# chaoyang223/UDA

Measured on AMD Instinct MI355X. Metric: TeraSort shuffle+merge GB/s whole-node, higher is better.
Workload: dtype bytes

## Files before the change

csrc/gpu/colpack.hip:

```cpp
#include "codec/colpack.h"
#include "kernels.h"

#include <algorithm>

namespace uda {
namespace gpu {

namespace {
constexpr int kCpThreads = 256;
constexpr int kCpTileRows = 128;
constexpr int kCpTileBytes = kCpTileRows * (9 * kColpackMaxRecordBytes / 10);
constexpr int kCpTableDelta = 2 * kColpackMaxRecordBytes;
constexpr int kCpTableStride = kCpTableDelta + 2 * kColpackMaxKeyBytes;

__device__ __forceinline__ uint64_t load_cols(const uint8_t* p, int n) {
  if (n == 8 && (reinterpret_cast<uintptr_t>(p) & 7) == 0) return *reinterpret_cast<const uint64_t*>(p);
  uint64_t x = 0;
  for (int k = 0; k < n; ++k) x |= (uint64_t)p[k] << (8 * k);
  return x;
}

struct Key128 {
  uint64_t hi, lo;
};
// ... 29 lines not shown
#pragma unroll
  for (int c = 0; c < 8; ++c) {
    const int col = 8 * g + c;
    if (col >= ko && col < ko + kl) {
      const int j = ko + kl - 1 - col;
      const uint64_t b = (j < 8 ? t.lo >> (8 * j) : t.hi >> (8 * (j - 8))) & 0xFF;
      x = (x & ~(0xFFull << (8 * c))) | (b << (8 * c));
    }
  }
  return x;
}

__device__ __forceinline__ bool group_has_key(int g, int ko, int kl) { return kl > 0 && 8 * g < ko + kl && 8 * g + 8 > ko; }

__global__ void __launch_bounds__(kCpThreads) colpack_stats_kernel(const ColpackPieceDesc* pieces, int L,
                                                                   uint32_t buf_records, int ko, int kl,
                                                                   uint32_t* table) {
  const ColpackPieceDesc pc = pieces[blockIdx.y];
  const int G = (L + 7) / 8;
  const int rows_per_iter = kCpThreads / G;
  if ((int64_t)blockIdx.x * rows_per_iter >= pc.nrec) return;
  __shared__ uint32_t s_mn[kColpackMaxRecordBytes], s_mx[kColpackMaxRecordBytes];
  __shared__ uint32_t s_dmn[kColpackMaxKeyBytes], s_dmx[kColpackMaxKeyBytes];
  const int t = threadIdx.x;
  s_mn[t] = 255;
  s_mx[t] = 0;
  if (t < kColpackMaxKeyBytes) {
    s_dmn[t] = 255;
    s_dmx[t] = 0;
  }
  __syncthreads();
  const int g = t % G, rl = t / G;
  if (rl < rows_per_iter) {
    const int ncol = min(8, L - 8 * g);
    const bool keyed = group_has_key(g, ko, kl);
    uint32_t mn[8], mx[8], dmn[8], dmx[8];
#pragma unroll
    for (int c = 0; c < 8; ++c) {
      mn[c] = dmn[c] = 255;
      mx[c] = dmx[c] = 0;
    }
    const uint8_t* p = pc.src + 8 * g;
    const int64_t step = (int64_t)gridDim.x * rows_per_iter;
#pragma unroll 4
    for (int64_t r = (int64_t)blockIdx.x * rows_per_iter + rl; r < pc.nrec; r += step) {
      const uint64_t x = load_cols(p + r * L, ncol);
#pragma unroll
      for (int c = 0; c < 8; ++c) {
        const uint32_t v = (uint32_t)(x >> (8 * c)) & 0xFF;
        mn[c] = min(mn[c], v);
        mx[c] = max(mx[c], v);
      }
      if (keyed) {
        const uint64_t xd = with_key_delta(x, g, key_delta(pc.src + r * L, r, L, buf_records, ko, kl), ko, kl);
#pragma unroll
        for (int c = 0; c < 8; ++c) {
          const uint32_t v = (uint32_t)(xd >> (8 * c)) & 0xFF;
          dmn[c] = min(dmn[c], v);
          dmx[c] = max(dmx[c], v);
        }
      }
    }
#pragma unroll
    for (int c = 0; c < 8; ++c)
      if (c < ncol) {
        atomicMin(&s_mn[8 * g + c], mn[c]);
        atomicMax(&s_mx[8 * g + c], mx[c]);
        const int kc = 8 * g + c - ko;
        if (keyed && kc >= 0 && kc < kl) {
          atomicMin(&s_dmn[kc], dmn[c]);
          atomicMax(&s_dmx[kc], dmx[c]);
        }
      }
  }
  __syncthreads();
  uint32_t* tb = table + (size_t)blockIdx.y * kCpTableStride;
  if (t < L) {
    atomicMin(&tb[t], s_mn[t]);
    atomicMin(&tb[kColpackMaxRecordBytes + t], 255u - s_mx[t]);
  }
  if (t < kl) {
    atomicMin(&tb[kCpTableDelta + t], s_dmn[t]);
    atomicMin(&tb[kCpTableDelta + kColpackMaxKeyBytes + t], 255u - s_dmx[t]);
  }
}

__device__ __forceinline__ int width_of(uint32_t mn, uint32_t mx) {
  const uint32_t range = mx > mn ? mx - mn : 0;
  return range ? 32 - __clz((int)range) : 0;
}

__global__ void __launch_bounds__(64) colpack_plan_kernel(const ColpackPieceDesc* pieces, int L, uint32_t buf_records,
                                                          uint32_t version, int ko, int kl, const uint32_t* table,
                                                          ColpackResult* results) {
  const ColpackPieceDesc pc = pieces[blockIdx.x];
  const uint32_t* tb = table + (size_t)blockIdx.x * kCpTableStride;
// ... 158 lines not shown

void launch_colpack(const ColpackPieceDesc* pieces, int npieces, int64_t max_nrec, int L, int64_t buf_records,
                    uint32_t* table, ColpackResult* results, hipStream_t s, int version, int key_off, int key_len) {
  if (npieces <= 0) return;
  if (version != (int)kColpackVersion2) version = (int)kColpackVersion, key_len = 0;
  if (key_len <= 0 || key_len > kColpackMaxKeyBytes || key_off < 0 || key_off + key_len > L || buf_records < 1 ||
      buf_records > 0xFFFFFFFFll)
    key_len = 0;
  if (key_len == 0) key_off = 0;
  (void)hipMemsetAsync(table, 0xFF, colpack_table_bytes(npieces), s);
  const int G = (L + 7) / 8;
  const int rows_per_iter = kCpThreads / G;
  int64_t sb = (max_nrec + (int64_t)rows_per_iter * 32 - 1) / ((int64_t)rows_per_iter * 32);
  sb = std::max<int64_t>(1, std::min<int64_t>(sb, 256));
  hipLaunchKernelGGL(colpack_stats_kernel, dim3((unsigned)sb, (unsigned)npieces), dim3(kCpThreads), 0, s, pieces, L,
                     (uint32_t)buf_records, key_off, key_len, table);
  hipLaunchKernelGGL(colpack_plan_kernel, dim3((unsigned)npieces), dim3(64), 0, s, pieces, L, (uint32_t)buf_records,
                     (uint32_t)version, key_off, key_len, table, results);
  int64_t pb = (max_nrec + kCpTileRows - 1) / kCpTileRows;
  pb = std::max<int64_t>(1, std::min<int64_t>(pb, 1024));
  if (G == 13)
    hipLaunchKernelGGL(colpack_pack_kernel<13>, dim3((unsigned)pb, (unsigned)npieces), dim3(kCpThreads), 0, s, pieces, L);
  else
    hipLaunchKernelGGL(colpack_pack_kernel<0>, dim3((unsigned)pb, (unsigned)npieces), dim3(kCpThreads), 0, s, pieces, L);
}

}
}
```

csrc/gpu/delivery_schedule.cc:

```cpp
#include "delivery_schedule.h"

#include <algorithm>
#include <stdexcept>

namespace uda {
namespace gpu {

void check_delivery_order(const std::string& order) {
  if (order != "wave" && order != "reducer") throw std::runtime_error("delivery_order must be wave or reducer");
}

std::vector<DeliveryPiece> delivery_schedule(const std::vector<int64_t>& group_recs, int64_t piece_bytes,
                                             const std::string& order, int64_t record_bytes) {
  check_delivery_order(order);
  if (record_bytes < 1) throw std::runtime_error("delivery_schedule: record_bytes < 1");
  const int64_t piece = std::max<int64_t>(1, piece_bytes / record_bytes) * record_bytes;
  std::vector<DeliveryPiece> v;
  std::vector<size_t> first(group_recs.size() + 1, 0);
  int64_t goff = 0;
  size_t waves = 0;
  for (size_t i = 0; i < group_recs.size(); ++i) {
    if (group_recs[i] < 0) throw std::runtime_error("delivery_schedule: negative record count");
    const int64_t bytes = group_recs[i] * record_bytes;
    for (int64_t off = 0; off < bytes;) {
      const int64_t len = std::min(piece, bytes - off);
      off += len;
      v.push_back(DeliveryPiece{(int)i, goff + off - len, len, (int)v.size(), off >= bytes});
    }
    goff += bytes;
    first[i + 1] = v.size();
    waves = std::max(waves, first[i + 1] - first[i]);
  }
  if (order == "reducer") return v;
  std::vector<DeliveryPiece> w;
  w.reserve(v.size());
  for (size_t k = 0; k < waves; ++k)
    for (size_t i = 0; i < group_recs.size(); ++i)
      if (first[i] + k < first[i + 1]) w.push_back(v[first[i] + k]);
  return w;
}

}
}
```

csrc/gpu/delivery_schedule.h:

```cpp
#pragma once
#include <cstdint>
#include <string>
#include <vector>

namespace uda {
namespace gpu {

struct DeliveryPiece {
  int reducer;
  int64_t src_off;
  int64_t len;
  int pack_index;
  bool last_of_reducer;
};

void check_delivery_order(const std::string& order);

std::vector<DeliveryPiece> delivery_schedule(const std::vector<int64_t>& group_recs, int64_t piece_bytes,
                                             const std::string& order, int64_t record_bytes = 104);

}
}
```

csrc/gpu/device_engine.cc:

```cpp
#include "device_engine.h"
#include "codec/colpack.h"
#include "device_ptr.h"
#include "hbm_ledger.h"
#include "merge_plan.h"
#include "sdma.h"
#include "uda/fault.h"
#include "uda/topology.h"
#include "uda/trace.h"

#include <rccl/rccl.h>
#include <unistd.h>

#include <algorithm>
#include <atomic>
#include <chrono>
#include <cstring>
#include <map>
#include <mutex>
#include <numeric>
#include <stdexcept>

#include "uda/log.h"
#include "uda/vint.h"
#include "uda/thread_name.h"
// ... 694 lines not shown
}

ShuffleJob::ShuffleJob(const ShuffleConfig& cfg) : cfg_(cfg) {
  if (cfg_.world < 1 || cfg_.rank < 0 || cfg_.rank >= cfg_.world)
    throw std::runtime_error("ShuffleJob: bad rank/world");
  if (cfg_.maps_per_rank < 1) throw std::runtime_error("ShuffleJob: maps_per_rank < 1");
  if (cfg_.rounds < 1) cfg_.rounds = 1;
  if (cfg_.reducers < 1) cfg_.reducers = 1;
  if (cfg_.pinned_slots < 2) cfg_.pinned_slots = 2;
  if (cfg_.d2h != "sdma" && cfg_.d2h != "hip") throw std::runtime_error("ShuffleJob: d2h must be sdma or hip");
  if (cfg_.store != "hbm" && cfg_.store != "host" && cfg_.store != "disk")
    throw std::runtime_error("unknown store tier " + cfg_.store);
  if (cfg_.delivery_pack != "auto" && cfg_.delivery_pack != "v1" && cfg_.delivery_pack != "off")
    throw std::runtime_error("ShuffleJob: delivery_pack must be auto, v1 or off");
  check_delivery_order(cfg_.delivery_order);
  pack_ = cfg_.deliver_host && cfg_.delivery_pack != "off";
  pack_version_ = cfg_.delivery_pack == "v1" ? (int)kColpackVersion : (int)kColpackVersion2;
  if (const char* e = std::getenv("UDA_DELIVERY_PACK"))
    if (std::atoi(e) == 0) pack_ = false;
  R_ = cfg_.reducers;
  Q_ = cfg_.rounds;
  C_ = R_ * Q_;
  if ((int64_t)R_ * cfg_.world * cfg_.maps_per_rank > 65536)
    throw std::runtime_error("ShuffleJob: reducers * world * maps_per_rank must be <= 65536 (merge run index)");
  HIP_CHECK(hipSetDevice(cfg_.device));
  int lo_prio = 0, hi_prio = 0;
  HIP_CHECK(hipDeviceGetStreamPriorityRange(&lo_prio, &hi_prio));
  const bool spill = cfg_.store != "hbm";
  HIP_CHECK(hipStreamCreateWithPriority(&s_comm_, hipStreamNonBlocking, spill ? lo_prio : hi_prio));
  HIP_CHECK(hipStreamCreateWithPriority(&s_compute_, hipStreamNonBlocking, spill ? hi_prio : lo_prio));
  HIP_CHECK(hipStreamCreateWithFlags(&s_copy_, hipStreamNonBlocking));
  HIP_CHECK(hipStreamCreateWithFlags(&s_plan_, hipStreamNonBlocking));
  buf_records_ = std::max<int64_t>(1, cfg_.kv_buf_bytes / kTeraRecordBytes);
  const int64_t buf_bytes = buf_records_ * kTeraRecordBytes;
  piece_bytes_ = std::max<int64_t>(1, cfg_.d2h_piece_bytes / buf_bytes) * buf_bytes;
  ring_stride_ = pack_ ? std::max(piece_bytes_, pack_bound(piece_bytes_ / kTeraRecordBytes)) : piece_bytes_;
  merged_ev_.resize(kSlots);
  comm_ev_.resize(kSlots);
  sent_ev_.resize(2);
  early_ev_.resize(kSlots);
  for (auto& e : early_ev_) HIP_CHECK(hipEventCreateWithFlags(&e, hipEventDisableTiming));
  for (auto& e : merged_ev_) HIP_CHECK(hipEventCreateWithFlags(&e, hipEventDisableTiming));
  for (auto& e : comm_ev_) HIP_CHECK(hipEventCreateWithFlags(&e, hipEventDisableTiming));
  for (auto& e : sent_ev_) HIP_CHECK(hipEventCreateWithFlags(&e, hipEventDisableTiming));
}

ShuffleJob::~ShuffleJob() {
  {
    std::lock_guard<std::mutex> g(mu_);
    stop_ = true;
  }
  cv_.notify_all();
  if (copy_thr_.joinable()) copy_thr_.join();
  for (auto& t : consumers_)
    if (t.joinable()) t.join();
  (void)hipDeviceSynchronize();
  for (auto e : merged_ev_) (void)hipEventDestroy(e);
  for (auto e : early_ev_) (void)hipEventDestroy(e);
  if (s_stage_) (void)hipStreamDestroy(s_stage_);
  for (auto e : comm_ev_) (void)hipEventDestroy(e);
  for (auto e : sent_ev_) (void)hipEventDestroy(e);
  for (auto e : piece_ev_) (void)hipEventDestroy(e);
  if (!sdma_ && ring_) pinned_host_free(ring_);
  if (sdma_) {
    for (auto sg : piece_sig_) sdma_->destroy_signal(sg);
    sdma_->free_host(ring_);
    ring_ = nullptr;
    sdma_.reset();
  }
  exchange_.reset();
  if (s_copy_) (void)hipStreamDestroy(s_copy_);
  if (s_plan_) (void)hipStreamDestroy(s_plan_);
  if (s_comm_) (void)hipStreamDestroy(s_comm_);
// ... 10 lines not shown
  if (cfg_.world == 1) return;
  if (cfg_.local_group.empty()) throw std::runtime_error("init_local: config.local_group is empty");
  HIP_CHECK(hipSetDevice(cfg_.device));
  exchange_ = make_local_exchange(cfg_.local_group, cfg_.rank, cfg_.world);
}

void ShuffleJob::init_ipc(const std::string& name) {
  if (cfg_.world == 1) return;
  HIP_CHECK(hipSetDevice(cfg_.device));
  exchange_ = make_ipc_exchange(name, cfg_.rank, cfg_.world, cfg_.device);
}

std::string ShuffleJob::delivery_name() const {
  if (!cfg_.deliver_host) return "none";
  std::string name = sdma_ ? sdma_->describe() : "hip[numa=" + std::to_string(device_numa_node(cfg_.device)) + "]";
  name += " ring=" + ring_numa_ + " order=" + cfg_.delivery_order;
  if (!pack_) return name + " pack=off";
  name += " pack=colbits v" + std::to_string(pack_version_);
  if (last_delta_ >= 0) name += last_delta_ ? " delta" : " plain";
  if (last_d2h_ratio_ >= 0) {
    char b[32];
    std::snprintf(b, sizeof(b), " d2h/in=%.3f", last_d2h_ratio_);
    name += b;
  }
  return name;
}

int64_t ShuffleJob::pack_bound(int64_t nrec) const {
  return pack_version_ == (int)kColpackVersion ? colpack_bound(kTeraRecordBytes, nrec)
                                               : colpack2_bound(kTeraRecordBytes, nrec, buf_records_);
}

std::vector<ShuffleJob::PackPiece> ShuffleJob::round_pieces(const std::vector<int64_t>& group_recs) const {
  std::vector<PackPiece> v;
  int64_t doff = 0;
  for (const DeliveryPiece& dp : delivery_schedule(group_recs, piece_bytes_, "reducer", kTeraRecordBytes)) {
    const int64_t nrec = dp.len / kTeraRecordBytes;
    v.push_back(PackPiece{dp.src_off, doff, nrec});
    doff += pack_bound(nrec);
  }
  return v;
}

void ShuffleJob::note_issue(int k, double now) {
  if (first_issue_ms_ < 0) first_issue_ms_ = now;
  if (flying_ == 0 && idle_since_ms_ >= 0) step_link_idle_ms_ += now - idle_since_ms_;
  slot_flying_[k] = true;
  ++flying_;
}

void ShuffleJob::note_landing(int k, double now) {
// ... 416 lines not shown
      }
      verify_n_[q] = (int)vruns[q].size();
    }
  }

  merger_.reset(new DeviceMerger(max_round_records_, R_ * W * M));
  const size_t out_bytes = (size_t)std::max<int64_t>(1, max_round_records_) * kTeraRecordBytes;
  out_slots_.clear();
  out_slots_.resize(kSlots);
  for (auto& b : out_slots_) b.alloc(out_bytes);
  packed_slots_.clear();
  d_pack_pieces_.clear();
  d_pack_results_.clear();
  h_pack_results_.clear();
  pack_n_.assign(Q_, 0);
  pack_max_nrec_.assign(Q_, 0);
  pack_early_.assign(Q_, 0);
  if (pack_) {
    int64_t packed_bytes = 64;
    int max_pieces = 1;
    std::vector<std::vector<PackPiece>> pieces(Q_);
    for (int q = 0; q < Q_; ++q) {
      pieces[q] = round_pieces(plans_[q].group_recs);
      if (pieces[q].size() > 65535) throw std::runtime_error("delivery_pack: more than 65535 D2H pieces in a round");
      pack_n_[q] = (int)pieces[q].size();
      max_pieces = std::max(max_pieces, pack_n_[q]);
      for (const PackPiece& pc : pieces[q]) {
        pack_max_nrec_[q] = std::max(pack_max_nrec_[q], pc.nrec);
        packed_bytes = std::max(packed_bytes, pc.dst_off + pack_bound(pc.nrec));
      }
    }
    packed_slots_.resize(kSlots);
    for (auto& b : packed_slots_) b.alloc((size_t)packed_bytes);
    d_pack_results_.resize(kSlots);
    h_pack_results_.resize(kSlots);
    for (int k = 0; k < kSlots; ++k) {
      d_pack_results_[k].alloc((size_t)max_pieces * sizeof(ColpackResult));
      h_pack_results_[k].alloc((size_t)max_pieces * sizeof(ColpackResult));
    }
    d_pack_table_.alloc(colpack_table_bytes(max_pieces));
    d_pack_pieces_.resize(Q_);
    for (int q = 0; q < Q_; ++q) {
      if (pieces[q].empty()) continue;
      std::vector<ColpackPieceDesc> v;
      int wave0 = 0;
      for (const DeliveryPiece& dp :
           delivery_schedule(plans_[q].group_recs, piece_bytes_, cfg_.delivery_order, kTeraRecordBytes)) {
        const PackPiece& pc = pieces[q][(size_t)dp.pack_index];
        v.push_back(ColpackPieceDesc{out_slots_[q % kSlots].as<uint8_t>() + pc.src_off,
                                     packed_slots_[q % kSlots].as<uint8_t>() + pc.dst_off, pc.nrec});
      }
      for (int64_t g : plans_[q].group_recs) wave0 += g > 0 ? 1 : 0;
      if (cfg_.delivery_order == "wave" && wave0 < pack_n_[q]) pack_early_[q] = wave0;
      d_pack_pieces_[q].alloc(v.size() * sizeof(ColpackPieceDesc));
      HIP_CHECK(hipMemcpy(d_pack_pieces_[q].as(), v.data(), v.size() * sizeof(ColpackPieceDesc), hipMemcpyHostToDevice));
    }
  }
  recv_slots_.clear();
  if (staged()) {
    recv_slots_.resize(kSlots);
    for (auto& b : recv_slots_) b.alloc((size_t)std::max<int64_t>(max_slot_bytes, 16));
  }
  for (auto& b : send_staging_) b.reset();
  if (W > 1 && spilled())
    for (auto& b : send_staging_) b.alloc((size_t)std::max<int64_t>(max_send, 16));
  if (W > 1) exchange_->reserve(max_send);
  for (int q = 0; q < Q_; ++q) {
    RoundPlan& rp = plans_[q];
// ... 156 lines not shown
}

void ShuffleJob::copy_loop() {
  try {
    bind_thread_to_cpus(device_consumer_cpus(cfg_.device));
    HIP_CHECK(hipSetDevice(cfg_.device));
    for (;;) {
      RoundOut r;
      {
        std::unique_lock<std::mutex> lk(mu_);
        cv_.wait(lk, [&] { return stop_ || !round_q_.empty(); });
        if (stop_) return;
        r = std::move(round_q_.front());
        round_q_.pop_front();
      }
      HIP_CHECK(hipEventSynchronize(r.early > 0 ? early_ev_[r.slot] : merged_ev_[r.slot]));
      const uint8_t* src = out_slots_[r.slot].as<uint8_t>();
      const bool last_round = (r.q == Q_ - 1);
      bool check;
      {
        std::lock_guard<std::mutex> g(mu_);
        check = step_check_delivery_;
      }
      if (check) {
        std::vector<RunDesc> gr(R_);
        int64_t o = 0, mx = 0;
        for (int i = 0; i < R_; ++i) {
          gr[i].base = src + o * kTeraRecordBytes;
          gr[i].nrec = r.group_recs[i];
          gr[i].nbytes = gr[i].nrec * kTeraRecordBytes;
          gr[i].offsets = nullptr;
          o += r.group_recs[i];
          mx = std::max(mx, r.group_recs[i]);
        }
        std::vector<uint64_t> ck(R_, 0);
        HIP_CHECK(hipMemcpyAsync(d_d2h_runs_.as(), gr.data(), (size_t)R_ * sizeof(RunDesc), hipMemcpyHostToDevice, s_copy_));
        launch_slice_checksums(d_d2h_runs_.as<RunDesc>(), R_, std::max<int64_t>(mx, 1),
                               d_d2h_ck_.as<unsigned long long>(), s_copy_);
        HIP_CHECK(hipGetLastError());
        HIP_CHECK(hipMemcpyAsync(ck.data(), d_d2h_ck_.as(), (size_t)R_ * 8, hipMemcpyDeviceToHost, s_copy_));
        HIP_CHECK(hipStreamSynchronize(s_copy_));
        std::lock_guard<std::mutex> g(mu_);
        for (int i = 0; i < R_; ++i) pre_d2h_ck_[(size_t)r.q * R_ + i] = ck[i];
      }
      std::vector<int> used;
      const std::vector<PackPiece> ppieces = pack_ ? round_pieces(r.group_recs) : std::vector<PackPiece>();
      const ColpackResult* pres = pack_ ? h_pack_results_[r.slot].as<ColpackResult>() : nullptr;
      if (last_round) {
        bool any = false;
        {
          std::lock_guard<std::mutex> g(mu_);
          for (int i = 0; i < R_; ++i)
            if (r.group_recs[i] == 0) {
              items_[i].push_back(Item{-1, 0, true, now_ms(), r.q});
              any = true;
            }
        }
        if (any) cv_.notify_all();
      }
      int issued = 0;
      for (const DeliveryPiece& dp :
           delivery_schedule(r.group_recs, piece_bytes_, cfg_.delivery_order, kTeraRecordBytes)) {
        if (r.early > 0 && issued == r.early) HIP_CHECK(hipEventSynchronize(merged_ev_[r.slot]));
        int k = -1;
        {
          std::unique_lock<std::mutex> lk(mu_);
          auto have_slot = [&] {
            if (stop_) return true;
            for (bool f : pinned_free_)
              if (f) return true;
            return false;
          };
          if (!have_slot()) {
            const double tw = now_ms();
            while (!cv_.wait_for(lk, std::chrono::microseconds(200), have_slot)) poll_landings();
            step_slot_wait_ms_ += now_ms() - tw;
          }
          if (stop_) return;
// ... 546 lines not shown
      int64_t goff = 0;
      for (int i = 0; i < R_; ++i) {
        const int64_t g = rp.group_recs[i];
        if (g > 0) {
          launch_validate_fixed(out + goff * kTeraRecordBytes, g, vprev + i, has_prev[i] ? 1 : 0, vlast + i, vstats,
                                s_compute_, dg + 4 + i);
          HIP_CHECK(hipMemcpyAsync(vprev + i, vlast + i, sizeof(Elem), hipMemcpyDeviceToDevice, s_compute_));
          has_prev[i] = true;
        }
        goff += g;
      }
      check_inputs(1);
    }
    HIP_CHECK(hipEventRecord(ev[4 * q + 3], s_compute_));
    if (pack_ && deliver && pack_n_[q] > 0) {
      auto pack_range = [&](int a, int b) {
        launch_colpack(d_pack_pieces_[q].as<ColpackPieceDesc>() + a, b - a, pack_max_nrec_[q], kTeraRecordBytes,
                       buf_records_, d_pack_table_.as<uint32_t>(), d_pack_results_[slot].as<ColpackResult>() + a,
                       s_compute_, pack_version_, kTeraKeyOffset, kTeraKeyBytes);
        HIP_CHECK(hipGetLastError());
        HIP_CHECK(hipMemcpyAsync(h_pack_results_[slot].as<ColpackResult>() + a,
                                 d_pack_results_[slot].as<ColpackResult>() + a, (size_t)(b - a) * sizeof(ColpackResult),
                                 hipMemcpyDeviceToHost, s_compute_));
      };
      if (pack_early_[q] > 0) {
        pack_range(0, pack_early_[q]);
        HIP_CHECK(hipEventRecord(early_ev_[slot], s_compute_));
      }
      pack_range(pack_early_[q], pack_n_[q]);
    }
    HIP_CHECK(hipEventRecord(merged_ev_[slot], s_compute_));
    if (sdma_stage) {
      std::lock_guard<std::mutex> g(mu_);
      merge_recorded[q] = 1;
      cv_.notify_all();
    }
    st.records += n;
    if (deliver) {
      {
        std::lock_guard<std::mutex> g(mu_);
        round_q_.push_back(RoundOut{q, slot, rp.group_recs, pack_early_[q]});
      }
      cv_.notify_all();
    }
  }
  if (deliver) wait_until([&] { return eof_count_ == R_; });
  if (exchange_) exchange_->wait(s_comm_);
  HIP_CHECK(hipStreamSynchronize(s_compute_));
  HIP_CHECK(hipStreamSynchronize(s_comm_));
  HIP_CHECK(hipStreamSynchronize(s_copy_));
  if (stage_thr.joinable()) stage_thr.join();
  if (exchange_) exchange_->quiesce();
  st.wall_ms = now_ms() - t0;
  st.stage_ms = stage_ms;
  for (int q = 0; q < Q_; ++q) {
    float a = 0, b = 0;
// ... 55 lines not shown
```

csrc/gpu/device_engine.h:

```cpp
#pragma once
#include <hip/hip_runtime.h>

#include <atomic>
#include <condition_variable>
#include <cstdint>
#include <deque>
#include <functional>
#include <map>
#include <memory>
#include <mutex>
#include <string>
#include <thread>
#include <vector>

#include "delivery_schedule.h"
#include "exchange.h"
#include "kernels.h"
#include "disk_store.h"
#include "sdma.h"

namespace uda {
namespace gpu {

void hip_check(hipError_t e, const char* what, const char* file, int line);
// ... 181 lines not shown
  int64_t kv_buf_bytes = 1 << 20;
  int64_t d2h_piece_bytes = 128ll << 20;
  int pinned_slots = 16;
  int d2h_engines = 1;
  std::string d2h = "sdma";
  bool deliver_host = true;
  bool validate = false;
  std::string local_group;
  std::string store = "hbm";
  std::string local_dirs;
  bool replan = false;
  bool map_sort = false;
  bool check_delivery = false;
  std::string delivery_pack = "auto";
  std::string delivery_order = "wave";
};

struct StepStats {
  double wall_ms = 0;
  double comm_ms = 0;
  double merge_ms = 0;
  double d2h_ms = 0;
  double wait_out_ms = 0;
  double plan_ms = 0;
  double stage_ms = 0;
  int64_t bytes_in = 0;
  int64_t records = 0;
  int64_t bytes_sent = 0;
  int64_t bytes_h2d = 0;
  int64_t buffers = 0;
// ... 131 lines not shown
  bool step_check_delivery_ = false;
  DeviceBuffer d_d2h_runs_, d_d2h_ck_;
  std::vector<DeviceBuffer> h2d_descs_;
  std::vector<int> h2d_n_;
  std::vector<int64_t> h2d_max_;
  int h2d_blocks_ = 2048;
  bool sdma_h2d_ = true;
  hipStream_t s_stage_ = nullptr;
  int64_t buf_records_ = 0;
  int64_t piece_bytes_ = 0;
  struct PackPiece {
    int64_t src_off;
    int64_t dst_off;
    int64_t nrec;
  };
  std::vector<PackPiece> round_pieces(const std::vector<int64_t>& group_recs) const;
  int64_t pack_bound(int64_t nrec) const;
  bool pack_ = false;
  int pack_version_ = 2;
  std::vector<DeviceBuffer> packed_slots_;
  std::vector<DeviceBuffer> d_pack_pieces_;
  std::vector<int> pack_n_;
  std::vector<int> pack_early_;
  std::vector<hipEvent_t> early_ev_;
  std::vector<int64_t> pack_max_nrec_;
  DeviceBuffer d_pack_table_;
  std::vector<DeviceBuffer> d_pack_results_;
  std::vector<PinnedBuffer> h_pack_results_;
  int64_t ring_stride_ = 0;
  double last_d2h_ratio_ = -1;
  int last_delta_ = -1;

  std::unique_ptr<SdmaEngine> sdma_;
  uint8_t* ring_ = nullptr;
  std::string ring_numa_;
  std::vector<hsa_signal_t> piece_sig_;
  std::vector<hipEvent_t> piece_ev_;
  struct RoundOut {
    int q;
    int slot;
    std::vector<int64_t> group_recs;
    int early = 0;
  };
  struct Item {
    int pslot;
    int64_t bytes;
    bool last;
    double issued_ms;
    int q;
    bool packed = false;
    int64_t copied = 0;
  };
  std::mutex mu_;
  std::condition_variable cv_;
  std::deque<RoundOut> round_q_;
  std::vector<std::deque<Item>> items_;
  std::vector<bool> pinned_free_;
// ... 35 lines not shown
```

csrc/python/bindings.cc:

```cpp
#include <map>
#include <memory>
#include <condition_variable>
#include <mutex>
#include <pybind11/functional.h>
#include <pybind11/numpy.h>
#include <pybind11/pybind11.h>
#include <pybind11/stl.h>

#include <fcntl.h>
#include <unistd.h>

#include <atomic>
#include <chrono>
#include <cstring>

#include "block_decoder.h"
#include "device_engine.h"
#include "device_ptr.h"
#include "mof_cache.h"
#include "consumer/reduce_task.h"
#include "service/merge_service.h"
#include "exchange.h"
#include "api_bench.h"
#include "generic_merger.h"
// ... 90 lines not shown
  get("kv_buf_bytes", c.kv_buf_bytes);
  get("d2h_piece_bytes", c.d2h_piece_bytes);
  get("pinned_slots", c.pinned_slots);
  get("d2h_engines", c.d2h_engines);
  get("d2h", c.d2h);
  get("deliver_host", c.deliver_host);
  get("validate", c.validate);
  get("local_group", c.local_group);
  get("store", c.store);
  get("local_dirs", c.local_dirs);
  get("replan", c.replan);
  get("map_sort", c.map_sort);
  get("check_delivery", c.check_delivery);
  get("delivery_pack", c.delivery_pack);
  get("delivery_order", c.delivery_order);
  return c;
}

struct PyBridge {
  py::object fetch_over, data_from_uda, get_path, get_conf, log, failure;
  uda_handle* h = nullptr;
  std::vector<std::shared_ptr<std::string>> keep;

  static PyBridge* self(void* ctx) { return static_cast<PyBridge*>(ctx); }
  static void t_fetch_over(void* ctx) {
    py::gil_scoped_acquire g;
    try {
      if (!self(ctx)->fetch_over.is_none()) self(ctx)->fetch_over();
    } catch (py::error_already_set& e) {
      e.discard_as_unraisable("fetch_over");
// ... 197 lines not shown
  m.def("delivery_schedule", [](const std::vector<int64_t>& group_recs, int64_t piece_bytes, const std::string& order,
                                int64_t record_bytes) {
    if (order != "wave" && order != "reducer") throw py::value_error("delivery_order must be wave or reducer");
    py::list out;
    for (const gpu::DeliveryPiece& p : gpu::delivery_schedule(group_recs, piece_bytes, order, record_bytes)) {
      py::dict d;
      d["reducer"] = p.reducer;
      d["src_off"] = p.src_off;
      d["len"] = p.len;
      d["pack_index"] = p.pack_index;
      d["last_of_reducer"] = p.last_of_reducer;
      out.append(d);
    }
    return out;
  }, py::arg("group_recs"), py::arg("piece_bytes"), py::arg("order") = "wave", py::arg("record_bytes") = 104);
  m.def("colpack_header_bytes", [] { return (int64_t)kColpackHeaderBytes; });
  m.def("colpack_have_bmi2", &colpack_have_bmi2);
  m.def("colpack_encode", [](py::bytes b, int L, int64_t buf_records) {
    std::string s = b;
    if (L < 1 || L > kColpackMaxRecordBytes || s.empty() || s.size() % (size_t)L)
      throw py::value_error("colpack_encode: need whole records of 1..256 bytes");
    const int64_t nrec = (int64_t)s.size() / L;
    std::string out((size_t)colpack_bound(L, nrec), '\0');
    const int64_t n = colpack_encode((const uint8_t*)s.data(), nrec, L, buf_records, (uint8_t*)&out[0]);
    out.resize((size_t)n);
    return py::bytes(out);
  }, py::arg("records"), py::arg("record_bytes"), py::arg("buf_records") = 1);
  m.def("colpack2_encode", [](py::bytes b, int L, int64_t buf_records, int key_off, int key_len) {
    std::string s = b;
    if (L < 1 || L > kColpackMaxRecordBytes || s.empty() || s.size() % (size_t)L)
// ... 1280 lines not shown
```

uda_amd/models/terasort.py:

```python
from __future__ import annotations

import dataclasses
import os
import sys
import secrets
import time

import numpy as np

from .._native import native
from ..parallel.dist import DistContext
from ..parallel.plan import round_bounds

RECORD_BYTES = 104
TERAGEN_ROW_BYTES = 100


@dataclasses.dataclass
class TeraSortConfig:
    rows_per_gpu: int = 1_250_000_000
    maps_per_rank: int = 32
    rounds: int = 16
    seed: int = 0x5EED
    kv_buf_bytes: int = 1 << 20
    reducers: int = 1
    d2h_piece_bytes: int = 128 << 20
    pinned_slots: int = 16
    d2h_engines: int = 1
    d2h: str = "sdma"
    deliver_host: bool = True
    validate: bool = False
    sample_every: int = 4096
    store: str = "hbm"
    local_dirs: str = "/tmp"
    replan: bool = False
    map_sort: bool = False
    check_delivery: bool = False
    delivery_pack: str = "auto"
    delivery_order: str = "wave"
    exchange: str = "ipc"


class TeraSortShuffle:
    def __init__(self, ctx: DistContext, cfg: TeraSortConfig, device: int | None = None):
        self.ctx = ctx
        self.cfg = cfg
        self.device = ctx.local_rank if device is None else device
        n = native()
        records_per_map = max(1, cfg.rows_per_gpu // cfg.maps_per_rank)
        self.records_per_map = records_per_map
        self.job = n.ShuffleJob(dict(
            device=self.device, rank=ctx.rank, world=ctx.world,
            maps_per_rank=cfg.maps_per_rank, records_per_map=records_per_map,
            rounds=cfg.rounds, reducers=cfg.reducers, seed=cfg.seed, kv_buf_bytes=cfg.kv_buf_bytes,
            d2h_piece_bytes=cfg.d2h_piece_bytes, pinned_slots=cfg.pinned_slots,
            d2h_engines=cfg.d2h_engines, d2h=cfg.d2h, deliver_host=cfg.deliver_host,
            validate=cfg.validate, store=cfg.store, local_dirs=cfg.local_dirs, replan=cfg.replan,
            map_sort=cfg.map_sort, check_delivery=cfg.check_delivery,
            delivery_pack=cfg.delivery_pack, delivery_order=cfg.delivery_order))
        self.sink = n.J2CSink(cfg.reducers, cfg.kv_buf_bytes)
        self.sampler = None
        self.sample_index = []
        self.expected_checksum = None
        self.expected_records = None
        self.setup_s = {}

    def setup(self) -> None:
        n = native()
        t0 = time.perf_counter()
        if self.ctx.world > 1:
            if self.cfg.exchange == "ipc" and not self._ipc_preflight():
                if os.environ.get("UDA_IPC_FALLBACK", "1") == "0":
                    raise RuntimeError(f"IPC exchange preflight failed ({self.ipc_fallback}); the job stops here "
                                       "(UDA_IPC_FALLBACK=0)")
# ... 122 lines not shown
        if stats["checksum"] != expected_checksum:
            raise AssertionError("checksum mismatch " + stats.get("diag", ""))


def make_local_group(world: int, cfg: TeraSortConfig, device: int = 0, group: str = "local"):

    n = native()
    records_per_map = max(1, cfg.rows_per_gpu // cfg.maps_per_rank)
    jobs = [n.ShuffleJob(dict(
        device=device, rank=r, world=world, maps_per_rank=cfg.maps_per_rank,
        records_per_map=records_per_map, rounds=cfg.rounds, reducers=cfg.reducers, seed=cfg.seed,
        kv_buf_bytes=cfg.kv_buf_bytes, d2h_piece_bytes=cfg.d2h_piece_bytes, pinned_slots=cfg.pinned_slots,
        d2h_engines=cfg.d2h_engines, d2h=cfg.d2h, deliver_host=cfg.deliver_host, validate=cfg.validate,
        local_group=group, store=cfg.store, local_dirs=cfg.local_dirs, replan=cfg.replan,
        map_sort=cfg.map_sort, check_delivery=cfg.check_delivery,
        delivery_pack=cfg.delivery_pack, delivery_order=cfg.delivery_order))
        for r in range(world)]
    for j in jobs:
        j.init_local()
        j.generate()
    local = [j.sample_keys(cfg.sample_every) for j in jobs]
    per_dest = []
    for d in range(world):
        parts = [np.asarray(s[d]) for s in local if np.asarray(s[d]).size]
        per_dest.append(np.concatenate(parts) if parts else np.zeros((0, 2), np.uint64))
    bounds = np.ascontiguousarray(round_bounds(per_dest, cfg.rounds * cfg.reducers).reshape(-1))
    for j in jobs:
        j.set_bounds(bounds)
    run_collective(jobs, lambda j: j.plan())
    ck = [sum(j.local_dest_checksums()[d] for j in jobs) % (1 << 64) for d in range(world)]
    rec = [sum(j.local_dest_records()[d] for j in jobs) for d in range(world)]
# ... 24 lines not shown
```

Baseline: 91.94.

## Taper delivery pieces at round edges, pack per wave, split key-delta stats kernel

On the first round, delivery pieces now start small and grow geometrically; on the last round they shrink again toward the end. The aim is to shorten pipeline fill and drain around host delivery. Column packing is launched once per delivery wave with its own event, so D2H of early waves can start before later waves are packed, replacing the single early/late split. Key-delta statistics move into a separate kernel that computes 128-bit key differences using wavefront shuffles instead of per-group reconstruction. The cost is more small pieces, more kernel launches and events, and more host synchronisation points.

```diff
diff --git a/csrc/gpu/colpack.hip b/csrc/gpu/colpack.hip
--- a/csrc/gpu/colpack.hip
+++ b/csrc/gpu/colpack.hip
@@ -67,31 +67,24 @@
 __device__ __forceinline__ bool group_has_key(int g, int ko, int kl) { return kl > 0 && 8 * g < ko + kl && 8 * g + 8 > ko; }
 
 __global__ void __launch_bounds__(kCpThreads) colpack_stats_kernel(const ColpackPieceDesc* pieces, int L,
-                                                                   uint32_t buf_records, int ko, int kl,
                                                                    uint32_t* table) {
   const ColpackPieceDesc pc = pieces[blockIdx.y];
   const int G = (L + 7) / 8;
   const int rows_per_iter = kCpThreads / G;
   if ((int64_t)blockIdx.x * rows_per_iter >= pc.nrec) return;
   __shared__ uint32_t s_mn[kColpackMaxRecordBytes], s_mx[kColpackMaxRecordBytes];
-  __shared__ uint32_t s_dmn[kColpackMaxKeyBytes], s_dmx[kColpackMaxKeyBytes];
   const int t = threadIdx.x;
   s_mn[t] = 255;
   s_mx[t] = 0;
-  if (t < kColpackMaxKeyBytes) {
-    s_dmn[t] = 255;
-    s_dmx[t] = 0;
-  }
   __syncthreads();
   const int g = t % G, rl = t / G;
   if (rl < rows_per_iter) {
     const int ncol = min(8, L - 8 * g);
-    const bool keyed = group_has_key(g, ko, kl);
-    uint32_t mn[8], mx[8], dmn[8], dmx[8];
+    uint32_t mn[8], mx[8];
 #pragma unroll
     for (int c = 0; c < 8; ++c) {
-      mn[c] = dmn[c] = 255;
-      mx[c] = dmx[c] = 0;
+      mn[c] = 255;
+      mx[c] = 0;
     }
     const uint8_t* p = pc.src + 8 * g;
     const int64_t step = (int64_t)gridDim.x * rows_per_iter;
@@ -104,35 +97,92 @@
         mn[c] = min(mn[c], v);
         mx[c] = max(mx[c], v);
       }
-      if (keyed) {
-        const uint64_t xd = with_key_delta(x, g, key_delta(pc.src + r * L, r, L, buf_records, ko, kl), ko, kl);
-#pragma unroll
-        for (int c = 0; c < 8; ++c) {
-          const uint32_t v = (uint32_t)(xd >> (8 * c)) & 0xFF;
-          dmn[c] = min(dmn[c], v);
-          dmx[c] = max(dmx[c], v);
-        }
-      }
     }
 #pragma unroll
     for (int c = 0; c < 8; ++c)
       if (c < ncol) {
         atomicMin(&s_mn[8 * g + c], mn[c]);
         atomicMax(&s_mx[8 * g + c], mx[c]);
-        const int kc = 8 * g + c - ko;
-        if (keyed && kc >= 0 && kc < kl) {
-          atomicMin(&s_dmn[kc], dmn[c]);
-          atomicMax(&s_dmx[kc], dmx[c]);
-        }
-      }
-  }
-  __syncthreads();
-  uint32_t* tb = table + (size_t)blockIdx.y * kCpTableStride;
+      }
+  }
+  __syncthreads();
   if (t < L) {
+    uint32_t* tb = table + (size_t)blockIdx.y * kCpTableStride;
     atomicMin(&tb[t], s_mn[t]);
     atomicMin(&tb[kColpackMaxRecordBytes + t], 255u - s_mx[t]);
   }
+}
+
+__device__ __forceinline__ Key128 load_key_words(const uint8_t* rec, int L, int ko, int kl) {
+  const int g0 = ko >> 3, g1 = (ko + kl - 1) >> 3;
+  uint64_t w[3] = {0, 0, 0};
+#pragma unroll
+  for (int k = 0; k < 3; ++k)
+    if (g0 + k <= g1) w[k] = load_cols(rec + 8 * (g0 + k), min(8, L - 8 * (g0 + k)));
+  const int s = 8 * (ko & 7);
+  const uint64_t a = s ? (w[0] >> s) | (w[1] << (64 - s)) : w[0];
+  const uint64_t b = s ? (w[1] >> s) | (w[2] << (64 - s)) : w[1];
+  uint64_t hi = __builtin_bswap64(a), lo = __builtin_bswap64(b);
+  const int drop = 8 * (kColpackMaxKeyBytes - kl);
+  if (drop >= 64) {
+    lo = hi >> (drop - 64);
+    hi = 0;
+  } else if (drop) {
+    lo = (lo >> drop) | (hi << (64 - drop));
+    hi >>= drop;
+  }
+  return Key128{hi, lo};
+}
+
+__global__ void __launch_bounds__(kCpThreads) colpack_keystats_kernel(const ColpackPieceDesc* pieces, int L,
+                                                                      uint32_t buf_records, int ko, int kl,
+                                                                      uint32_t* table) {
+  const ColpackPieceDesc pc = pieces[blockIdx.y];
+  if ((int64_t)blockIdx.x * kCpThreads >= pc.nrec) return;
+  __shared__ uint32_t s_dmn[kColpackMaxKeyBytes], s_dmx[kColpackMaxKeyBytes];
+  const int t = threadIdx.x;
+  if (t < kColpackMaxKeyBytes) {
+    s_dmn[t] = 255;
+    s_dmx[t] = 0;
+  }
+  __syncthreads();
+  uint32_t dmn[kColpackMaxKeyBytes], dmx[kColpackMaxKeyBytes];
+#pragma unroll
+  for (int j = 0; j < kColpackMaxKeyBytes; ++j) {
+    dmn[j] = 255;
+    dmx[j] = 0;
+  }
+  const int64_t step = (int64_t)gridDim.x * kCpThreads;
+  for (int64_t base = (int64_t)blockIdx.x * kCpThreads + (t & ~63); base < pc.nrec; base += step) {
+    const int64_t r = base + (t & 63);
+    const bool valid = r < pc.nrec;
+    const uint8_t* rec = pc.src + (valid ? r : base) * L;
+    const Key128 k = load_key_words(rec, L, ko, kl);
+    Key128 prev;
+    prev.hi = __shfl_up((unsigned long long)k.hi, 1);
+    prev.lo = __shfl_up((unsigned long long)k.lo, 1);
+    const bool restart = is_restart(r, buf_records);
+    if ((t & 63) == 0 && !restart) prev = load_key_words(rec - L, L, ko, kl);
+    if (valid) {
+      const uint64_t lo = restart ? 0 : k.lo - prev.lo;
+      const uint64_t hi = restart ? 0 : k.hi - prev.hi - (k.lo < prev.lo ? 1 : 0);
+#pragma unroll
+      for (int j = 0; j < kColpackMaxKeyBytes; ++j) {
+        const uint32_t v = (uint32_t)((j < 8 ? lo >> (8 * j) : hi >> (8 * (j - 8))) & 0xFF);
+        dmn[j] = min(dmn[j], v);
+        dmx[j] = max(dmx[j], v);
+      }
+    }
+  }
+#pragma unroll
+  for (int j = 0; j < kColpackMaxKeyBytes; ++j)
+    if (j < kl) {
+      atomicMin(&s_dmn[kl - 1 - j], dmn[j]);
+      atomicMax(&s_dmx[kl - 1 - j], dmx[j]);
+    }
+  __syncthreads();
   if (t < kl) {
+    uint32_t* tb = table + (size_t)blockIdx.y * kCpTableStride;
     atomicMin(&tb[kCpTableDelta + t], s_dmn[t]);
     atomicMin(&tb[kCpTableDelta + kColpackMaxKeyBytes + t], 255u - s_dmx[t]);
   }
@@ -321,7 +371,13 @@
   int64_t sb = (max_nrec + (int64_t)rows_per_iter * 32 - 1) / ((int64_t)rows_per_iter * 32);
   sb = std::max<int64_t>(1, std::min<int64_t>(sb, 256));
   hipLaunchKernelGGL(colpack_stats_kernel, dim3((unsigned)sb, (unsigned)npieces), dim3(kCpThreads), 0, s, pieces, L,
-                     (uint32_t)buf_records, key_off, key_len, table);
+                     table);
+  if (key_len > 0) {
+    int64_t kb = (max_nrec + (int64_t)kCpThreads * 32 - 1) / ((int64_t)kCpThreads * 32);
+    kb = std::max<int64_t>(1, std::min<int64_t>(kb, 256));
+    hipLaunchKernelGGL(colpack_keystats_kernel, dim3((unsigned)kb, (unsigned)npieces), dim3(kCpThreads), 0, s, pieces,
+                       L, (uint32_t)buf_records, key_off, key_len, table);
+  }
   hipLaunchKernelGGL(colpack_plan_kernel, dim3((unsigned)npieces), dim3(64), 0, s, pieces, L, (uint32_t)buf_records,
                      (uint32_t)version, key_off, key_len, table, results);
   int64_t pb = (max_nrec + kCpTileRows - 1) / kCpTileRows;
diff --git a/csrc/gpu/delivery_schedule.cc b/csrc/gpu/delivery_schedule.cc
--- a/csrc/gpu/delivery_schedule.cc
+++ b/csrc/gpu/delivery_schedule.cc
@@ -10,11 +10,52 @@
   if (order != "wave" && order != "reducer") throw std::runtime_error("delivery_order must be wave or reducer");
 }
 
-std::vector<DeliveryPiece> delivery_schedule(const std::vector<int64_t>& group_recs, int64_t piece_bytes,
-                                             const std::string& order, int64_t record_bytes) {
+void check_delivery_taper(const std::string& taper) {
+  if (taper != "auto" && taper != "off") throw std::runtime_error("delivery_taper must be auto or off");
+}
+
+namespace {
+std::vector<int64_t> taper_sizes(int64_t piece_bufs, int64_t p0, double grow) {
+  std::vector<int64_t> v;
+  double x = (double)p0;
+  while (x < (double)piece_bufs) {
+    v.push_back(std::max<int64_t>(1, (int64_t)x));
+    x *= grow;
+  }
+  return v;
+}
+}
+
+std::vector<int64_t> taper_cell_bufs(int64_t nbuf, int64_t piece_bufs, const DeliveryTaper& t) {
+  if (piece_bufs < 1 || t.p0 < 1) throw std::runtime_error("delivery taper: piece and p0 must be at least one buffer");
+  if ((t.head && !(t.grow_head > 1.0)) || (t.tail && !(t.grow_tail > 1.0)))
+    throw std::runtime_error("delivery taper: growth factors must exceed 1");
+  std::vector<int64_t> head = t.head ? taper_sizes(piece_bufs, t.p0, t.grow_head) : std::vector<int64_t>();
+  std::vector<int64_t> tail = t.tail ? taper_sizes(piece_bufs, t.p0, t.grow_tail) : std::vector<int64_t>();
+  int64_t used = 0;
+  for (int64_t s : head) used += s;
+  for (int64_t s : tail) used += s;
+  while (used > nbuf) {
+    std::vector<int64_t>& from = tail.empty() ? head : tail;
+    used -= from.back();
+    from.pop_back();
+  }
+  std::vector<int64_t> v = head;
+  int64_t mid = nbuf - used;
+  for (; mid >= piece_bufs; mid -= piece_bufs) v.push_back(piece_bufs);
+  if (mid > 0) v.push_back(mid);
+  v.insert(v.end(), tail.rbegin(), tail.rend());
+  return v;
+}
+
+std::vector<DeliveryPiece> delivery_schedule_tapered(const std::vector<int64_t>& group_recs, int64_t piece_bytes,
+                                                     const std::string& order, int64_t record_bytes,
+                                                     const DeliveryTaper& taper) {
   check_delivery_order(order);
   if (record_bytes < 1) throw std::runtime_error("delivery_schedule: record_bytes < 1");
   const int64_t piece = std::max<int64_t>(1, piece_bytes / record_bytes) * record_bytes;
+  const int64_t buf = taper.buf_bytes;
+  const bool tapered = (taper.head || taper.tail) && buf > 0 && buf % record_bytes == 0 && piece % buf == 0;
   std::vector<DeliveryPiece> v;
   std::vector<size_t> first(group_recs.size() + 1, 0);
   int64_t goff = 0;
@@ -22,10 +63,19 @@
   for (size_t i = 0; i < group_recs.size(); ++i) {
     if (group_recs[i] < 0) throw std::runtime_error("delivery_schedule: negative record count");
     const int64_t bytes = group_recs[i] * record_bytes;
-    for (int64_t off = 0; off < bytes;) {
-      const int64_t len = std::min(piece, bytes - off);
-      off += len;
-      v.push_back(DeliveryPiece{(int)i, goff + off - len, len, (int)v.size(), off >= bytes});
+    if (tapered) {
+      int64_t off = 0;
+      for (int64_t nb : taper_cell_bufs((bytes + buf - 1) / buf, piece / buf, taper)) {
+        const int64_t len = std::min(nb * buf, bytes - off);
+        off += len;
+        v.push_back(DeliveryPiece{(int)i, goff + off - len, len, (int)v.size(), off >= bytes});
+      }
+    } else {
+      for (int64_t off = 0; off < bytes;) {
+        const int64_t len = std::min(piece, bytes - off);
+        off += len;
+        v.push_back(DeliveryPiece{(int)i, goff + off - len, len, (int)v.size(), off >= bytes});
+      }
     }
     goff += bytes;
     first[i + 1] = v.size();
@@ -40,5 +90,10 @@
   return w;
 }
 
+std::vector<DeliveryPiece> delivery_schedule(const std::vector<int64_t>& group_recs, int64_t piece_bytes,
+                                             const std::string& order, int64_t record_bytes) {
+  return delivery_schedule_tapered(group_recs, piece_bytes, order, record_bytes, DeliveryTaper());
+}
+
 }
 }
diff --git a/csrc/gpu/delivery_schedule.h b/csrc/gpu/delivery_schedule.h
--- a/csrc/gpu/delivery_schedule.h
+++ b/csrc/gpu/delivery_schedule.h
@@ -19,5 +19,22 @@
 std::vector<DeliveryPiece> delivery_schedule(const std::vector<int64_t>& group_recs, int64_t piece_bytes,
                                              const std::string& order, int64_t record_bytes = 104);
 
+struct DeliveryTaper {
+  int64_t buf_bytes = 0;
+  bool head = false;
+  bool tail = false;
+  int64_t p0 = 4;
+  double grow_head = 3.0;
+  double grow_tail = 2.0;
+};
+
+void check_delivery_taper(const std::string& taper);
+
+std::vector<int64_t> taper_cell_bufs(int64_t nbuf, int64_t piece_bufs, const DeliveryTaper& t);
+
+std::vector<DeliveryPiece> delivery_schedule_tapered(const std::vector<int64_t>& group_recs, int64_t piece_bytes,
+                                                     const std::string& order, int64_t record_bytes,
+                                                     const DeliveryTaper& taper);
+
 }
 }
diff --git a/csrc/gpu/device_engine.cc b/csrc/gpu/device_engine.cc
--- a/csrc/gpu/device_engine.cc
+++ b/csrc/gpu/device_engine.cc
@@ -732,6 +732,7 @@
   if (cfg_.delivery_pack != "auto" && cfg_.delivery_pack != "v1" && cfg_.delivery_pack != "off")
     throw std::runtime_error("ShuffleJob: delivery_pack must be auto, v1 or off");
   check_delivery_order(cfg_.delivery_order);
+  check_delivery_taper(cfg_.delivery_taper);
   pack_ = cfg_.deliver_host && cfg_.delivery_pack != "off";
   pack_version_ = cfg_.delivery_pack == "v1" ? (int)kColpackVersion : (int)kColpackVersion2;
   if (const char* e = std::getenv("UDA_DELIVERY_PACK"))
@@ -756,8 +757,7 @@
   merged_ev_.resize(kSlots);
   comm_ev_.resize(kSlots);
   sent_ev_.resize(2);
-  early_ev_.resize(kSlots);
-  for (auto& e : early_ev_) HIP_CHECK(hipEventCreateWithFlags(&e, hipEventDisableTiming));
+  wave_ev_.resize(kSlots);
   for (auto& e : merged_ev_) HIP_CHECK(hipEventCreateWithFlags(&e, hipEventDisableTiming));
   for (auto& e : comm_ev_) HIP_CHECK(hipEventCreateWithFlags(&e, hipEventDisableTiming));
   for (auto& e : sent_ev_) HIP_CHECK(hipEventCreateWithFlags(&e, hipEventDisableTiming));
@@ -774,7 +774,8 @@
     if (t.joinable()) t.join();
   (void)hipDeviceSynchronize();
   for (auto e : merged_ev_) (void)hipEventDestroy(e);
-  for (auto e : early_ev_) (void)hipEventDestroy(e);
+  for (auto& v : wave_ev_)
+    for (auto e : v) (void)hipEventDestroy(e);
   if (s_stage_) (void)hipStreamDestroy(s_stage_);
   for (auto e : comm_ev_) (void)hipEventDestroy(e);
   for (auto e : sent_ev_) (void)hipEventDestroy(e);
@@ -815,7 +816,7 @@
 std::string ShuffleJob::delivery_name() const {
   if (!cfg_.deliver_host) return "none";
   std::string name = sdma_ ? sdma_->describe() : "hip[numa=" + std::to_string(device_numa_node(cfg_.device)) + "]";
-  name += " ring=" + ring_numa_ + " order=" + cfg_.delivery_order;
+  name += " ring=" + ring_numa_ + " order=" + cfg_.delivery_order + " taper=" + cfg_.delivery_taper;
   if (!pack_) return name + " pack=off";
   name += " pack=colbits v" + std::to_string(pack_version_);
   if (last_delta_ >= 0) name += last_delta_ ? " delta" : " plain";
@@ -832,10 +833,21 @@
                                                : colpack2_bound(kTeraRecordBytes, nrec, buf_records_);
 }
 
-std::vector<ShuffleJob::PackPiece> ShuffleJob::round_pieces(const std::vector<int64_t>& group_recs) const {
+std::vector<DeliveryPiece> ShuffleJob::round_schedule(int q, const std::vector<int64_t>& group_recs,
+                                                      const std::string& order) const {
+  DeliveryTaper t;
+  if (cfg_.delivery_taper != "off") {
+    t.buf_bytes = buf_records_ * kTeraRecordBytes;
+    t.head = q == 0;
+    t.tail = q == Q_ - 1;
+  }
+  return delivery_schedule_tapered(group_recs, piece_bytes_, order, kTeraRecordBytes, t);
+}
+
+std::vector<ShuffleJob::PackPiece> ShuffleJob::round_pieces(int q, const std::vector<int64_t>& group_recs) const {
   std::vector<PackPiece> v;
   int64_t doff = 0;
-  for (const DeliveryPiece& dp : delivery_schedule(group_recs, piece_bytes_, "reducer", kTeraRecordBytes)) {
+  for (const DeliveryPiece& dp : round_schedule(q, group_recs, "reducer")) {
     const int64_t nrec = dp.len / kTeraRecordBytes;
     v.push_back(PackPiece{dp.src_off, doff, nrec});
     doff += pack_bound(nrec);
@@ -1282,19 +1294,19 @@
   d_pack_results_.clear();
   h_pack_results_.clear();
   pack_n_.assign(Q_, 0);
-  pack_max_nrec_.assign(Q_, 0);
-  pack_early_.assign(Q_, 0);
+  pack_wave_.assign(Q_, {});
+  pack_wave_nrec_.assign(Q_, {});
   if (pack_) {
     int64_t packed_bytes = 64;
     int max_pieces = 1;
     std::vector<std::vector<PackPiece>> pieces(Q_);
     for (int q = 0; q < Q_; ++q) {
-      pieces[q] = round_pieces(plans_[q].group_recs);
+      pieces[q] = round_pieces(q, plans_[q].group_recs);
       if (pieces[q].size() > 65535) throw std::runtime_error("delivery_pack: more than 65535 D2H pieces in a round");
       pack_n_[q] = (int)pieces[q].size();
       max_pieces = std::max(max_pieces, pack_n_[q]);
       for (const PackPiece& pc : pieces[q]) {
-        pack_max_nrec_[q] = std::max(pack_max_nrec_[q], pc.nrec);
+        if (pack_bound(pc.nrec) > ring_stride_) throw std::runtime_error("delivery_pack: a piece's bound exceeds a ring slot");
         packed_bytes = std::max(packed_bytes, pc.dst_off + pack_bound(pc.nrec));
       }
     }
@@ -1311,15 +1323,24 @@
     for (int q = 0; q < Q_; ++q) {
       if (pieces[q].empty()) continue;
       std::vector<ColpackPieceDesc> v;
-      int wave0 = 0;
-      for (const DeliveryPiece& dp :
-           delivery_schedule(plans_[q].group_recs, piece_bytes_, cfg_.delivery_order, kTeraRecordBytes)) {
+      int prev_reducer = -1;
+      for (const DeliveryPiece& dp : round_schedule(q, plans_[q].group_recs, cfg_.delivery_order)) {
         const PackPiece& pc = pieces[q][(size_t)dp.pack_index];
+        if (v.empty() || (cfg_.delivery_order == "wave" && dp.reducer <= prev_reducer)) {
+          pack_wave_[q].push_back((int)v.size());
+          pack_wave_nrec_[q].push_back(0);
+        }
+        prev_reducer = dp.reducer;
+        pack_wave_nrec_[q].back() = std::max(pack_wave_nrec_[q].back(), pc.nrec);
         v.push_back(ColpackPieceDesc{out_slots_[q % kSlots].as<uint8_t>() + pc.src_off,
                                      packed_slots_[q % kSlots].as<uint8_t>() + pc.dst_off, pc.nrec});
       }
-      for (int64_t g : plans_[q].group_recs) wave0 += g > 0 ? 1 : 0;
-      if (cfg_.delivery_order == "wave" && wave0 < pack_n_[q]) pack_early_[q] = wave0;
+      pack_wave_[q].push_back((int)v.size());
+      for (auto& evs : wave_ev_)
+        while (evs.size() + 1 < pack_wave_[q].size()) {
+          evs.push_back(nullptr);
+          HIP_CHECK(hipEventCreateWithFlags(&evs.back(), hipEventDisableTiming));
+        }
       d_pack_pieces_[q].alloc(v.size() * sizeof(ColpackPieceDesc));
       HIP_CHECK(hipMemcpy(d_pack_pieces_[q].as(), v.data(), v.size() * sizeof(ColpackPieceDesc), hipMemcpyHostToDevice));
     }
@@ -1506,7 +1527,8 @@
         r = std::move(round_q_.front());
         round_q_.pop_front();
       }
-      HIP_CHECK(hipEventSynchronize(r.early > 0 ? early_ev_[r.slot] : merged_ev_[r.slot]));
+      const bool waves = pack_ && !pack_wave_[r.q].empty();
+      HIP_CHECK(hipEventSynchronize(waves ? wave_ev_[r.slot][0] : merged_ev_[r.slot]));
       const uint8_t* src = out_slots_[r.slot].as<uint8_t>();
       const bool last_round = (r.q == Q_ - 1);
       bool check;
@@ -1536,7 +1558,7 @@
         for (int i = 0; i < R_; ++i) pre_d2h_ck_[(size_t)r.q * R_ + i] = ck[i];
       }
       std::vector<int> used;
-      const std::vector<PackPiece> ppieces = pack_ ? round_pieces(r.group_recs) : std::vector<PackPiece>();
+      const std::vector<PackPiece> ppieces = pack_ ? round_pieces(r.q, r.group_recs) : std::vector<PackPiece>();
       const ColpackResult* pres = pack_ ? h_pack_results_[r.slot].as<ColpackResult>() : nullptr;
       if (last_round) {
         bool any = false;
@@ -1551,9 +1573,10 @@
         if (any) cv_.notify_all();
       }
       int issued = 0;
-      for (const DeliveryPiece& dp :
-           delivery_schedule(r.group_recs, piece_bytes_, cfg_.delivery_order, kTeraRecordBytes)) {
-        if (r.early > 0 && issued == r.early) HIP_CHECK(hipEventSynchronize(merged_ev_[r.slot]));
+      size_t wave = 1;
+      for (const DeliveryPiece& dp : round_schedule(r.q, r.group_recs, cfg_.delivery_order)) {
+        if (waves && wave + 1 < pack_wave_[r.q].size() && issued == pack_wave_[r.q][wave])
+          HIP_CHECK(hipEventSynchronize(wave_ev_[r.slot][wave++]));
         int k = -1;
         {
           std::unique_lock<std::mutex> lk(mu_);
@@ -2130,8 +2153,8 @@
     }
     HIP_CHECK(hipEventRecord(ev[4 * q + 3], s_compute_));
     if (pack_ && deliver && pack_n_[q] > 0) {
-      auto pack_range = [&](int a, int b) {
-        launch_colpack(d_pack_pieces_[q].as<ColpackPieceDesc>() + a, b - a, pack_max_nrec_[q], kTeraRecordBytes,
+      auto pack_range = [&](int a, int b, int64_t max_nrec) {
+        launch_colpack(d_pack_pieces_[q].as<ColpackPieceDesc>() + a, b - a, max_nrec, kTeraRecordBytes,
                        buf_records_, d_pack_table_.as<uint32_t>(), d_pack_results_[slot].as<ColpackResult>() + a,
                        s_compute_, pack_version_, kTeraKeyOffset, kTeraKeyBytes);
         HIP_CHECK(hipGetLastError());
@@ -2139,11 +2162,10 @@
                                  d_pack_results_[slot].as<ColpackResult>() + a, (size_t)(b - a) * sizeof(ColpackResult),
                                  hipMemcpyDeviceToHost, s_compute_));
       };
-      if (pack_early_[q] > 0) {
-        pack_range(0, pack_early_[q]);
-        HIP_CHECK(hipEventRecord(early_ev_[slot], s_compute_));
-      }
-      pack_range(pack_early_[q], pack_n_[q]);
+      for (size_t w = 0; w + 1 < pack_wave_[q].size(); ++w) {
+        pack_range(pack_wave_[q][w], pack_wave_[q][w + 1], pack_wave_nrec_[q][w]);
+        HIP_CHECK(hipEventRecord(wave_ev_[slot][w], s_compute_));
+      }
     }
     HIP_CHECK(hipEventRecord(merged_ev_[slot], s_compute_));
     if (sdma_stage) {
@@ -2155,7 +2177,7 @@
     if (deliver) {
       {
         std::lock_guard<std::mutex> g(mu_);
-        round_q_.push_back(RoundOut{q, slot, rp.group_recs, pack_early_[q]});
+        round_q_.push_back(RoundOut{q, slot, rp.group_recs});
       }
       cv_.notify_all();
     }
diff --git a/csrc/gpu/device_engine.h b/csrc/gpu/device_engine.h
--- a/csrc/gpu/device_engine.h
+++ b/csrc/gpu/device_engine.h
@@ -219,6 +219,7 @@
   bool check_delivery = false;
   std::string delivery_pack = "auto";
   std::string delivery_order = "wave";
+  std::string delivery_taper = "auto";
 };
 
 struct StepStats {
@@ -380,16 +381,18 @@
     int64_t dst_off;
     int64_t nrec;
   };
-  std::vector<PackPiece> round_pieces(const std::vector<int64_t>& group_recs) const;
+  std::vector<DeliveryPiece> round_schedule(int q, const std::vector<int64_t>& group_recs,
+                                            const std::string& order) const;
+  std::vector<PackPiece> round_pieces(int q, const std::vector<int64_t>& group_recs) const;
   int64_t pack_bound(int64_t nrec) const;
   bool pack_ = false;
   int pack_version_ = 2;
   std::vector<DeviceBuffer> packed_slots_;
   std::vector<DeviceBuffer> d_pack_pieces_;
   std::vector<int> pack_n_;
-  std::vector<int> pack_early_;
-  std::vector<hipEvent_t> early_ev_;
-  std::vector<int64_t> pack_max_nrec_;
+  std::vector<std::vector<int>> pack_wave_;
+  std::vector<std::vector<int64_t>> pack_wave_nrec_;
+  std::vector<std::vector<hipEvent_t>> wave_ev_;
   DeviceBuffer d_pack_table_;
   std::vector<DeviceBuffer> d_pack_results_;
   std::vector<PinnedBuffer> h_pack_results_;
@@ -406,7 +409,6 @@
     int q;
     int slot;
     std::vector<int64_t> group_recs;
-    int early = 0;
   };
   struct Item {
     int pslot;
diff --git a/csrc/python/bindings.cc b/csrc/python/bindings.cc
--- a/csrc/python/bindings.cc
+++ b/csrc/python/bindings.cc
@@ -128,6 +128,7 @@
   get("check_delivery", c.check_delivery);
   get("delivery_pack", c.delivery_pack);
   get("delivery_order", c.delivery_order);
+  get("delivery_taper", c.delivery_taper);
   return c;
 }
 
@@ -355,6 +356,36 @@
     }
     return out;
   }, py::arg("group_recs"), py::arg("piece_bytes"), py::arg("order") = "wave", py::arg("record_bytes") = 104);
+  m.def("delivery_schedule_tapered", [](const std::vector<int64_t>& group_recs, int64_t piece_bytes,
+                                        const std::string& order, int64_t record_bytes, int64_t buf_bytes, bool head,
+                                        bool tail, const std::string& taper, int64_t p0, double grow_head,
+                                        double grow_tail) {
+    if (order != "wave" && order != "reducer") throw py::value_error("delivery_order must be wave or reducer");
+    if (taper != "auto" && taper != "off") throw py::value_error("delivery_taper must be auto or off");
+    gpu::DeliveryTaper t;
+    if (taper == "auto") {
+      t.buf_bytes = buf_bytes;
+      t.head = head;
+      t.tail = tail;
+    }
+    t.p0 = p0;
+    t.grow_head = grow_head;
+    t.grow_tail = grow_tail;
+    py::list out;
+    for (const gpu::DeliveryPiece& p : gpu::delivery_schedule_tapered(group_recs, piece_bytes, order, record_bytes, t)) {
+      py::dict d;
+      d["reducer"] = p.reducer;
+      d["src_off"] = p.src_off;
+      d["len"] = p.len;
+      d["pack_index"] = p.pack_index;
+      d["last_of_reducer"] = p.last_of_reducer;
+      out.append(d);
+    }
+    return out;
+  }, py::arg("group_recs"), py::arg("piece_bytes"), py::arg("order") = "wave", py::arg("record_bytes") = 104,
+     py::arg("buf_bytes") = 0, py::arg("head") = false, py::arg("tail") = false, py::arg("taper") = "auto",
+     py::arg("p0") = gpu::DeliveryTaper().p0, py::arg("grow_head") = gpu::DeliveryTaper().grow_head,
+     py::arg("grow_tail") = gpu::DeliveryTaper().grow_tail);
   m.def("colpack_header_bytes", [] { return (int64_t)kColpackHeaderBytes; });
   m.def("colpack_have_bmi2", &colpack_have_bmi2);
   m.def("colpack_encode", [](py::bytes b, int L, int64_t buf_records) {
diff --git a/uda_amd/models/terasort.py b/uda_amd/models/terasort.py
--- a/uda_amd/models/terasort.py
+++ b/uda_amd/models/terasort.py
@@ -38,6 +38,7 @@
     check_delivery: bool = False
     delivery_pack: str = "auto"
     delivery_order: str = "wave"
+    delivery_taper: str = "auto"
     exchange: str = "ipc"
 
 
@@ -57,7 +58,8 @@
             d2h_engines=cfg.d2h_engines, d2h=cfg.d2h, deliver_host=cfg.deliver_host,
             validate=cfg.validate, store=cfg.store, local_dirs=cfg.local_dirs, replan=cfg.replan,
             map_sort=cfg.map_sort, check_delivery=cfg.check_delivery,
-            delivery_pack=cfg.delivery_pack, delivery_order=cfg.delivery_order))
+            delivery_pack=cfg.delivery_pack, delivery_order=cfg.delivery_order,
+            delivery_taper=cfg.delivery_taper))
         self.sink = n.J2CSink(cfg.reducers, cfg.kv_buf_bytes)
         self.sampler = None
         self.sample_index = []
@@ -210,7 +212,8 @@
         d2h_engines=cfg.d2h_engines, d2h=cfg.d2h, deliver_host=cfg.deliver_host, validate=cfg.validate,
         local_group=group, store=cfg.store, local_dirs=cfg.local_dirs, replan=cfg.replan,
         map_sort=cfg.map_sort, check_delivery=cfg.check_delivery,
-        delivery_pack=cfg.delivery_pack, delivery_order=cfg.delivery_order))
+        delivery_pack=cfg.delivery_pack, delivery_order=cfg.delivery_order,
+        delivery_taper=cfg.delivery_taper))
         for r in range(world)]
     for j in jobs:
         j.init_local()
```

Measured after the change: 91.34. Within noise of the previous version (-0.6%).
